# HKUDS/LLMRec

Hardware: NVIDIA H100
Metric: train_interactions_per_sec (higher is better)
Workload: dtype f32

## Files before the change

### llmrec_b200/csrc/proj_tc.cu

```cuda
#include <mutex>
#include <stdlib.h>
#include <vector>
#include <string.h>
#include "common.cuh"
#include "tc_common.cuh"
#include "proj_tc.cuh"

namespace llmrec {

using namespace tc;


typedef CUresult (*EncodeFn)(CUtensorMap*, CUtensorMapDataType, cuuint32_t, void*, const cuuint64_t*, const cuuint64_t*,
                             const cuuint32_t*, const cuuint32_t*, CUtensorMapInterleave, CUtensorMapSwizzle,
                             CUtensorMapL2promotion, CUtensorMapFloatOOBfill);

static EncodeFn get_encode() {
  static EncodeFn fn = nullptr;
  static bool tried = false;
  if (!tried) {
    tried = true;
    void* p = nullptr;
    cudaDriverEntryPointQueryResult q;
    if (cudaGetDriverEntryPoint("cuTensorMapEncodeTiled", &p, cudaEnableDefault, &q) == cudaSuccess && q == cudaDriverEntryPointSuccess)
// ... 54 lines not shown
  a[1] = lds_u32(row + 1024 + c0);
  a[2] = lds_u32(row + c1);
  a[3] = lds_u32(row + 1024 + c1);
}
__device__ __forceinline__ int wgrad_feature(int blk, int warp, int h, int g) {
  return blk * 64 + 32 * (warp >> 1) + 8 * (warp & 1) + 4 * h + (g & 3) + 16 * (g >> 2);
}
__device__ __forceinline__ void ld_frag_wgrad(uint32_t (&a)[4], uint32_t sx, int blk, int kk, int warp, int lane) {
  const int g = lane >> 2, t = lane & 3;
  const uint32_t base = sx + (blk * 2 + (warp >> 1)) * 4096 + kk * 1024 + t * 128 + (g & 3) * 4;
  const uint32_t q = (2 * (warp & 1) + 4 * (g >> 2)) ^ t;
  a[0] = lds_u32(base + (q << 4));
  a[1] = lds_u32(base + ((q ^ 1) << 4));
  a[2] = lds_u32(base + 512 + ((q ^ 4) << 4));
  a[3] = lds_u32(base + 512 + ((q ^ 5) << 4));
}

__device__ __forceinline__ uint32_t i8_pair_bf16(uint32_t w, int b, float s) {
  const float x0 = (__uint_as_float(__byte_perm(w, 0x4B000000u, 0x7650u + b)) - 8388736.0f) * s;
  const float x1 = (__uint_as_float(__byte_perm(w, 0x4B000000u, 0x7651u + b)) - 8388736.0f) * s;
  return __byte_perm(__float_as_uint(x0), __float_as_uint(x1), 0x7632u);
}
__device__ __forceinline__ void i8x16_bf16(const uint4& q, float s, uint4& lo, uint4& hi) {
  const uint32_t w0 = q.x ^ 0x80808080u, w1 = q.y ^ 0x80808080u, w2 = q.z ^ 0x80808080u, w3 = q.w ^ 0x80808080u;
  lo = make_uint4(i8_pair_bf16(w0, 0, s), i8_pair_bf16(w0, 2, s), i8_pair_bf16(w1, 0, s), i8_pair_bf16(w1, 2, s));
  hi = make_uint4(i8_pair_bf16(w2, 0, s), i8_pair_bf16(w2, 2, s), i8_pair_bf16(w3, 0, s), i8_pair_bf16(w3, 2, s));
}
__device__ __forceinline__ void converters_sync() { asm volatile("bar.sync 1, 96;" ::: "memory"); }

template <class Unit>
struct I8Stage {
  static constexpr int kGroups = Unit::Cfg::TM / 64, kTasks = 256;
  static constexpr int kPer = (kTasks + 95) / 96;
  float sc[kPer];
  const float* tile_sc = nullptr;
  __device__ void load_scales(const Unit& w, int kb, int ct) {
#pragma unroll
    for (int m = 0; m < kPer; ++m) {
      const int t = ct + 96 * m;
      sc[m] = t < kTasks ? w.row_scale(w.task_row(0, t, kb)) : 0.f;
    }
  }
  __device__ void expand(uint8_t* sx, int ct) const {
#pragma unroll
    for (int g = 0; g < kGroups; ++g) {
      uint4 v[kPer];
#pragma unroll
      for (int m = 0; m < kPer; ++m) {
        const int t = ct + 96 * m;
        if (t < kTasks) v[m] = *reinterpret_cast<const uint4*>(sx + Unit::Cfg::TM * 64u + g * 4096u + Unit::raw_off(t));
      }
      if (2 * g >= kGroups) converters_sync();
#pragma unroll
      for (int m = 0; m < kPer; ++m) {
        const int t = ct + 96 * m;
        if (t >= kTasks) continue;
        uint4 lo, hi;
        uint32_t o_lo, o_hi;
        i8x16_bf16(v[m], Unit::kScalesPerUnit ? tile_sc[64 * g + (t >> 2)] : sc[m], lo, hi);
        Unit::out_off(t, o_lo, o_hi);
        *reinterpret_cast<uint4*>(sx + g * 8192u + o_lo) = lo;
        *reinterpret_cast<uint4*>(sx + g * 8192u + o_hi) = hi;
      }
    }
  }
};

__device__ __forceinline__ uint32_t i8_raw_off(int t) { return (t >> 2) * 64u + (t & 3) * 16u; }
__device__ __forceinline__ void i8_out_off(int t, uint32_t& lo, uint32_t& hi) {
  const int i = t >> 2, c = 2 * (t & 3);
  lo = i * 128u + (((c ^ i) & 7) << 4);
  hi = i * 128u + ((((c + 1) ^ i) & 7) << 4);
}

__device__ __forceinline__ float i8_row_scale(const RowScales& xs, int p, int n, int row) {
  return row < n ? __ldg(reinterpret_cast<const float*>(xs.scale[p] + (long long)row * xs.pitch[p])) : 0.f;
}

template <int D, bool SPLIT, int MB, bool BF16 = false, bool I8 = false>
struct FwdUnit {
  using Cfg = ProjCfg<D, SPLIT, MB, BF16>;
  static_assert(!I8 || BF16, "int8 X runs the bf16 pipeline");
  static constexpr int kTransA = 0;
  static constexpr int kBuilders = I8 ? 3 : 0;
  static constexpr int kProducerRegs = I8 ? 72 : 40, kConsumerRegs = I8 ? 216 : 232;
  static constexpr uint32_t kRawTx = I8 ? Cfg::TM * 64u : 0u;
  static constexpr uint32_t kTx = I8 ? Cfg::kStage - Cfg::kX : Cfg::kStage;
  const FwdParams& P; int p, mblk, kb_n;
  __device__ FwdUnit(const FwdParams& P_, int u) : P(P_) {
    p = 0;
    while (p + 1 < P.n_prob && u >= P.prob[p + 1].tile_start) ++p;
    mblk = u - P.prob[p].tile_start;
    kb_n = P.prob[p].kblocks;
  }
  __device__ void issue(uint8_t* st, uint64_t* bar, uint64_t* raw_bar, int kb, uint64_t pol) const {
    constexpr int bk = stage_k(BF16);
    if constexpr (I8) tma_load_2d_hint(st + Cfg::TM * 64, &P.tmA[p], raw_bar, kb * bk, mblk * Cfg::TM, pol);
    else tma_load_2d_hint(st, &P.tmA[p], bar, kb * bk, mblk * Cfg::TM, pol);
#pragma unroll
    for (int i = 0; i < Cfg::NB; ++i) tma_load_2d(st + Cfg::kX + i * Cfg::kB, &P.tmW[p], bar, kb * bk, i * D);
  }
  static constexpr bool kScalesPerUnit = true;
  __device__ void tile_scales(float* ts, int ct) const {
    for (int i = ct; i < Cfg::TM; i += 96) ts[i] = i8_row_scale(P.xs, p, P.prob[p].n, mblk * Cfg::TM + i);
  }
  static __device__ uint32_t raw_off(int t) { return i8_raw_off(t); }
  static __device__ void out_off(int t, uint32_t& lo, uint32_t& hi) { i8_out_off(t, lo, hi); }
  static __device__ void ld_frag(uint32_t (&a)[4], uint32_t sx, int blk, int kk, int warp, int lane) { ld_frag_fwd(a, sx, blk, kk, warp, lane); }
  static __device__ uint64_t a_desc(uint32_t sx, int blk, int kk) { return gmma_desc_sw128(sx + blk * 8192u + kk * 32u); }
  __device__ void store(float (&acc)[MB][D / 2], int cw, int warp, int lane) const {
    const FwdProblem& pr = P.prob[p];
    const int g = lane >> 2, t = lane & 3;
#pragma unroll
    for (int j = 0; j < MB; ++j) {
      const int row0 = mblk * Cfg::TM + (cw * MB + j) * 64 + warp * 16 + g;
      long long yrow[2];
#pragma unroll
      for (int h = 0; h < 2; ++h) {
        const int row = row0 + 8 * h;
        yrow[h] = row < pr.n ? (pr.rows ? (long long)__ldg(pr.rows + row) : (long long)row) : -1;
      }
#pragma unroll
      for (int c = 0; c < D / 8; ++c) {
        const int col = c * 8 + 2 * t;
        const float2 b = pr.bias ? __ldg(reinterpret_cast<const float2*>(pr.bias + col)) : make_float2(0.f, 0.f);
#pragma unroll
        for (int h = 0; h < 2; ++h) {
          if (yrow[h] >= 0)
            *reinterpret_cast<float2*>(pr.Y + yrow[h] * pr.ldy + col) = make_float2(acc[j][4 * c + 2 * h] + b.x, acc[j][4 * c + 2 * h + 1] + b.y);
        }
      }
    }
  }
};

template <int D, bool SPLIT, int MB, bool BF16 = false, bool I8 = false>
struct WgUnit {
  using Cfg = ProjCfg<D, SPLIT, MB, BF16>;
  static_assert(!I8 || BF16, "int8 X runs the bf16 pipeline");
  static constexpr int kBk = stage_k(BF16);
  static constexpr int kTransA = 1;
  const WgParams& P; int p, u, ft, r0, kb_n;
  __device__ WgUnit(const WgParams& P_, int u_) : P(P_), u(u_) {
    p = 0;
    while (p + 1 < P.n_prob && u >= P.prob[p + 1].item_start) ++p;
    const WgProblem& pr = P.prob[p];
    const int local = u - pr.item_start, chunk = local / pr.ft_tiles;
    ft = local - chunk * pr.ft_tiles;
    r0 = chunk * pr.rows_per_chunk;
    kb_n = (min(pr.n, r0 + pr.rows_per_chunk) - r0 + kBk - 1) / kBk;
  }
  static constexpr bool kBuildsB = SPLIT && !BF16;
  static constexpr int kBuilders = kBuildsB || I8 ? 3 : 0;
  static constexpr int kProducerRegs = kBuilders ? 72 : 40;
  static constexpr int kConsumerRegs = kBuilders ? 216 : 232;
  static constexpr uint32_t kRawTx = I8 ? Cfg::TM * 64u : 0u;
  static constexpr uint32_t kTx = kBuildsB ? Cfg::kX : I8 ? Cfg::kStage - Cfg::kX : Cfg::kStage;
  __device__ void issue(uint8_t* st, uint64_t* bar, uint64_t* raw_bar, int kb, uint64_t pol) const {
    const int r = r0 + kb * kBk;
    if constexpr (I8) {
#pragma unroll
      for (int b = 0; b < Cfg::TM / 64; ++b) tma_load_2d_hint(st + Cfg::TM * 64 + b * 4096, &P.tmX[p], raw_bar, ft * Cfg::TM + 64 * b, r, pol);
    } else if constexpr (BF16) {
#pragma unroll
      for (int b = 0; b < Cfg::TM / 64; ++b) tma_load_2d_hint(st + b * 8192, &P.tmX[p], bar, ft * Cfg::TM + 64 * b, r, pol);
    } else {
#pragma unroll
      for (int b = 0; b < Cfg::TM / 32; ++b) tma_load_2d_hint(st + b * 4096, &P.tmX[p], bar, ft * Cfg::TM + 32 * b, r, pol);
    }
    if constexpr (!kBuildsB) {
#pragma unroll
      for (int i = 0; i < Cfg::NB; ++i) tma_load_2d(st + Cfg::kX + i * Cfg::kB, &P.tmG[p], bar, r, i * D);
    }
  }
  static constexpr bool kScalesPerUnit = false;
  __device__ void tile_scales(float*, int) const {}
  __device__ int task_row(int, int t, int kb) const { return r0 + kb * kBk + (t >> 2); }
  __device__ float row_scale(int row) const { return i8_row_scale(P.xs, p, P.prob[p].n, row); }
  static __device__ uint32_t raw_off(int t) { return i8_raw_off(t); }
  static __device__ void out_off(int t, uint32_t& lo, uint32_t& hi) { i8_out_off(t, lo, hi); }
  static constexpr int kTasks = D / 8;
  static constexpr int kBatch = 3;
  __device__ void build(uint8_t* st, int kb, int bw, int lane) const {
    const int n = P.prob[p].n, r = r0 + kb * kBk + lane;
    const int* __restrict__ map = P.rows[p];
    const float* src = r < n ? P.dY[p] + (long long)(map ? __ldg(map + r) : r) * P.lddy[p] : nullptr;
    uint8_t* b = st + Cfg::kX + (lane & 3) * 4;
    const int q = lane >> 2;
    for (int t0 = bw; t0 < kTasks; t0 += kBuilders * kBatch) {
      float4 v[kBatch][2];
#pragma unroll
      for (int j = 0; j < kBatch; ++j) {
        const int t = t0 + kBuilders * j;
#pragma unroll
        for (int h = 0; h < 2; ++h)
          v[j][h] = t < kTasks && src ? __ldg(reinterpret_cast<const float4*>(src + 8 * t + 4 * h)) : make_float4(0.f, 0.f, 0.f, 0.f);
      }
#pragma unroll
      for (int j = 0; j < kBatch; ++j) {
        const int t = t0 + kBuilders * j;
        if (t >= kTasks) break;
#pragma unroll
        for (int e = 0; e < 8; ++e) {
          const float4 w = v[j][e >> 2];
          const float x = (e & 3) == 0 ? w.x : (e & 3) == 1 ? w.y : (e & 3) == 2 ? w.z : w.w, hi = tf32_hi(x);
          uint8_t* o = b + (8 * t + e) * 128 + ((q ^ e) & 7) * 16;
          *reinterpret_cast<float*>(o) = hi;
          *reinterpret_cast<float*>(o + Cfg::kB) = x - hi;
        }
      }
    }
  }
  static __device__ void ld_frag(uint32_t (&a)[4], uint32_t sx, int blk, int kk, int warp, int lane) { ld_frag_wgrad(a, sx, blk, kk, warp, lane); }
  static __device__ uint64_t a_desc(uint32_t sx, int blk, int kk) { return gmma_desc_sw128_mn(sx + blk * 8192u + kk * 2048u); }
  __device__ void store(float (&acc)[MB][D / 2], int cw, int warp, int lane) const {
    const int g = lane >> 2, t = lane & 3;
    float* out = P.partial + (long long)u * Cfg::TM * D;
#pragma unroll
    for (int j = 0; j < MB; ++j)
#pragma unroll
      for (int h = 0; h < 2; ++h) {
        const int f = BF16 ? (cw * MB + j) * 64 + warp * 16 + 8 * h + g : wgrad_feature(cw * MB + j, warp, h, g);
        float* o = out + (long long)f * D + 2 * t;
#pragma unroll
        for (int c = 0; c < D / 8; ++c) *reinterpret_cast<float2*>(o + c * 8) = make_float2(acc[j][4 * c + 2 * h], acc[j][4 * c + 2 * h + 1]);
      }
  }
};

template <int D, bool SPLIT, int MB, bool BF16, class Unit, class Params>
__device__ __forceinline__ void proj_pipeline(const Params& P, int total) {
  using Cfg = ProjCfg<D, SPLIT, MB, BF16>;
  extern __shared__ uint8_t smem_raw[];
  uint8_t* smem = align1024(smem_raw);
  uint64_t* full = reinterpret_cast<uint64_t*>(smem + Cfg::kStages * Cfg::kStage);
  uint64_t* empty = full + Cfg::kStages;
  uint64_t* raw = empty + Cfg::kStages;
  float* tile_sc = reinterpret_cast<float*>(raw + Cfg::kStages);
  const int tid = threadIdx.x, wg = tid >> 7, warp = (tid >> 5) & 3, lane = tid & 31;
  if (tid == 0) {
    for (int s = 0; s < Cfg::kStages; ++s) { mbar_init(&full[s], 1 + Unit::kBuilders); mbar_init(&empty[s], 8); mbar_init(&raw[s], 1); }
    fence_barrier_init();
  }
  __syncthreads();

  static_assert(128 * Unit::kProducerRegs + 256 * Unit::kConsumerRegs <= 384 * 168, "setmaxnreg split exceeds the CTA's registers");
  if (wg == 0) {
    setmaxnreg_dec<Unit::kProducerRegs>();
    if (tid == 0) {
      const uint64_t pol = l2_policy_evict_first();
      int s = 0; uint32_t ph = 0;
      for (int u = blockIdx.x; u < total; u += gridDim.x) {
        const Unit w(P, u);
        for (int kb = 0; kb < w.kb_n; ++kb) {
          mbar_wait(&empty[s], ph ^ 1u);
          mbar_arrive_expect_tx(&full[s], Unit::kTx);
          if constexpr (Unit::kRawTx > 0) mbar_arrive_expect_tx(&raw[s], Unit::kRawTx);
          w.issue(smem + s * Cfg::kStage, &full[s], &raw[s], kb, pol);
          if (++s == Cfg::kStages) { s = 0; ph ^= 1u; }
        }
      }
    }
    if constexpr (Unit::kBuilders > 0) {
      if (warp >= 1) {
        int s = 0; uint32_t ph = 0;
        for (int u = blockIdx.x; u < total; u += gridDim.x) {
          const Unit w(P, u);
          [[maybe_unused]] I8Stage<Unit> cv;
          if constexpr (Unit::kRawTx > 0 && Unit::kScalesPerUnit) {
            converters_sync();
            w.tile_scales(tile_sc, tid - 32);
            converters_sync();
            cv.tile_sc = tile_sc;
          }
          for (int kb = 0; kb < w.kb_n; ++kb) {
            if constexpr (Unit::kRawTx > 0) {
              if constexpr (!Unit::kScalesPerUnit) cv.load_scales(w, kb, tid - 32);
              mbar_wait(&raw[s], ph);
              cv.expand(smem + s * Cfg::kStage, tid - 32);
            } else {
              mbar_wait(&empty[s], ph ^ 1u);
              w.build(smem + s * Cfg::kStage, kb, warp - 1, lane);
            }
            fence_proxy_async_smem();
            __syncwarp();
            if (lane == 0) mbar_arrive(&full[s]);
            if (++s == Cfg::kStages) { s = 0; ph ^= 1u; }
          }
        }
      }
    }
    return;
  }

  setmaxnreg_inc<Unit::kConsumerRegs>();
  const int cw = wg - 1;
  int s = 0; uint32_t ph = 0;
  float acc[MB][D / 2];
  for (int u = blockIdx.x; u < total; u += gridDim.x) {
    const Unit w(P, u);
#pragma unroll
    for (int j = 0; j < MB; ++j)
#pragma unroll
      for (int i = 0; i < D / 2; ++i) acc[j][i] = 0.f;
    int prev = -1;
    for (int kb = 0; kb < w.kb_n; ++kb) {
      mbar_wait(&full[s], ph);
      const uint32_t st = smem_u32(smem + s * Cfg::kStage), bh = st + Cfg::kX, bl = bh + Cfg::kB;
      if constexpr (BF16) {
#pragma unroll
        for (int kk = 0; kk < 4; ++kk) {
          wgmma_fence();
#pragma unroll
          for (int j = 0; j < MB; ++j) {
            const uint64_t a = Unit::a_desc(st, cw * MB + j, kk);
            if (SPLIT) {
              WgmmaSSbf16<D, Unit::kTransA>::mma(acc[j], a, gmma_desc_sw128(bl + Cfg::kB + kk * 32u));
              WgmmaSSbf16<D, Unit::kTransA>::mma(acc[j], a, gmma_desc_sw128(bl + kk * 32u));
            }
            WgmmaSSbf16<D, Unit::kTransA>::mma(acc[j], a, gmma_desc_sw128(bh + kk * 32u));
          }
          wgmma_commit();
          wgmma_wait<1>();
          if (kk == 0 && prev >= 0 && lane == 0) mbar_arrive(&empty[prev]);
        }
      } else {
#pragma unroll
        for (int kk = 0; kk < 4; ++kk) {
          uint32_t ah[MB][4], al[MB][4];
#pragma unroll
          for (int j = 0; j < MB; ++j) {
            Unit::ld_frag(ah[j], st, cw * MB + j, kk, warp, lane);
            if (SPLIT)
#pragma unroll
              for (int i = 0; i < 4; ++i) {
                const float x = __uint_as_float(ah[j][i]), hi = tf32_hi(x);
                ah[j][i] = __float_as_uint(hi);
                al[j][i] = __float_as_uint(x - hi);
              }
          }
          wgmma_fence();
          const uint64_t dh = gmma_desc_sw128(bh + kk * 32u);
#pragma unroll
          for (int j = 0; j < MB; ++j) {
            if (SPLIT) {
              WgmmaRS<D>::mma(acc[j], al[j], dh);
              WgmmaRS<D>::mma(acc[j], ah[j], gmma_desc_sw128(bl + kk * 32u));
            }
            WgmmaRS<D>::mma(acc[j], ah[j], dh);
          }
          wgmma_commit();
          wgmma_wait<1>();
          if (kk == 0 && prev >= 0 && lane == 0) mbar_arrive(&empty[prev]);
        }
      }
      prev = s;
      if (++s == Cfg::kStages) { s = 0; ph ^= 1u; }
    }
    wgmma_wait<0>();
    if (prev >= 0 && lane == 0) mbar_arrive(&empty[prev]);
    w.store(acc, cw, warp, lane);
  }
}

template <int D, bool SPLIT, int MB, XType XT>
__global__ void __launch_bounds__(384, 1) proj_fwd_tc_kernel(const __grid_constant__ FwdParams P) {
  constexpr bool BF16 = XT != XType::F32;
  proj_pipeline<D, SPLIT, MB, BF16, FwdUnit<D, SPLIT, MB, BF16, XT == XType::I8>>(P, P.total_tiles);
}

template <int D, bool SPLIT, int MB, XType XT>
__global__ void __launch_bounds__(384, 1) proj_wgrad_tc_kernel(const __grid_constant__ WgParams P) {
  constexpr bool BF16 = XT != XType::F32;
  proj_pipeline<D, SPLIT, MB, BF16, WgUnit<D, SPLIT, MB, BF16, XT == XType::I8>>(P, P.total_items);
}

static int num_sms() {
  static int n[64] = {};
  int dev = 0;
  if (cudaGetDevice(&dev) != cudaSuccess || dev < 0 || dev >= 64) return 132;
  if (!n[dev] && cudaDeviceGetAttribute(&n[dev], cudaDevAttrMultiProcessorCount, dev) != cudaSuccess) n[dev] = 132;
  return n[dev];
// ... 137 lines not shown
#pragma unroll 4
    for (int c = 0; c < pr.chunks; ++c, ++idx) {
      if ((idx & 3) != sl) continue;
      const float4 v = __ldg(reinterpret_cast<const float4*>(R.partial + ((long long)(pr.item_start + c * pr.ft_tiles + ft) * tm + f) * d) + dc4);
      s.x += v.x; s.y += v.y; s.z += v.z; s.w += v.w;
    }
  }
  part[sl][e] = s;
  __syncthreads();
  if (sl == 0 && owned) {
    float4 a = part[0][e], b = part[1][e], c = part[2][e], g = part[3][e];
    float4 t = make_float4((a.x + b.x) + (c.x + g.x), (a.y + b.y) + (c.y + g.y), (a.z + b.z) + (c.z + g.z), (a.w + b.w) + (c.w + g.w));
    const int gf = ft * tm + f;
    if (gf < ro.k) {
      float* p = ro.dW + (long long)(dc4 * 4) * ro.k + gf;
      if (ro.accumulate) { t.x += p[0]; t.y += p[ro.k]; t.z += p[2LL * ro.k]; t.w += p[3LL * ro.k]; }
      p[0] = t.x; p[ro.k] = t.y; p[2LL * ro.k] = t.z; p[3LL * ro.k] = t.w;
    }
  }
}

struct ColsumParams { const float* dY[kMaxProb]; long long ld[kMaxProb]; long long n[kMaxProb]; float* db[kMaxProb]; int acc[kMaxProb]; int d; int n_prob; float* partial; unsigned* ticket; };
constexpr int kColsumSlices = 128;
__global__ void __launch_bounds__(256) colsum_kernel(const ColsumParams P) {
  __shared__ float red[256];
  __shared__ bool s_last;
  const int p = blockIdx.y, b = blockIdx.x, d = P.d;
  const int groups = 256 / d > 0 ? 256 / d : 1;
  const int g = threadIdx.x / d, c = threadIdx.x - g * d;
  float s = 0.f;
  if (g < groups && P.db[p]) {
#pragma unroll 4
    for (long long r = (long long)b * groups + g; r < P.n[p]; r += (long long)kColsumSlices * groups) s += __ldg(P.dY[p] + r * P.ld[p] + c);
  }
  red[threadIdx.x] = (g < groups) ? s : 0.f;
  __syncthreads();
  if (threadIdx.x < d) {
    float t = 0.f;
    for (int gg = 0; gg < groups; ++gg) t += red[gg * d + threadIdx.x];
    P.partial[((long long)p * kColsumSlices + b) * d + threadIdx.x] = t;
  }
  __threadfence();
  __syncthreads();
  if (threadIdx.x == 0) s_last = atomicAdd(P.ticket, 1u) == gridDim.x * gridDim.y - 1;
  __syncthreads();
  if (!s_last) return;
  __threadfence();
  for (int q = 0; q < P.n_prob; ++q) {
    if (!P.db[q]) continue;
    float t = 0.f;
    if (g < groups)
      for (int bb = g; bb < kColsumSlices; bb += groups) t += __ldcg(P.partial + ((long long)q * kColsumSlices + bb) * d + c);
    __syncthreads();
    red[threadIdx.x] = (g < groups) ? t : 0.f;
    __syncthreads();
    if (threadIdx.x < d) {
      float u = 0.f;
      for (int gg = 0; gg < groups; ++gg) u += red[gg * d + threadIdx.x];
      float* o = P.db[q] + threadIdx.x;
      *o = P.acc[q] ? (*o + u) : u;
    }
  }
  if (threadIdx.x == 0) *P.ticket = 0u;
}

bool proj_tc_supported(int d, int64_t ldx, const void* X, int k, bool wgrad, XType xt) {
  (void)wgrad;
  const int q = xt == XType::I8 ? 16 : xt == XType::BF16 ? 8 : 4;
  return d % 32 == 0 && d >= 32 && d <= 256 && ldx % q == 0 && aligned16(X) && k >= 1 && k % q == 0;
}

static CUtensorMapDataType x_type(bool bf16) { return bf16 ? CU_TENSOR_MAP_DATA_TYPE_BFLOAT16 : CU_TENSOR_MAP_DATA_TYPE_FLOAT32; }

static bool x_tmap(CUtensorMap* m, XType xt, const void* X, int k, int64_t n, int64_t ldx, uint32_t box_k, uint32_t box_rows) {
  if (xt == XType::I8) return make_tmap_2d(m, CU_TENSOR_MAP_DATA_TYPE_UINT8, X, (uint64_t)k, (uint64_t)n, (uint64_t)ldx, box_k, box_rows, false);
  return make_tmap_2d(m, x_type(xt == XType::BF16), X, (uint64_t)k, (uint64_t)n, (uint64_t)ldx * (xt == XType::BF16 ? 2 : 4), box_k, box_rows);
}

static void set_row_scales(RowScales& xs, int p, XType xt, const void* X, int k, int64_t ldx) {
  xs.scale[p] = xt == XType::I8 ? static_cast<const uint8_t*>(X) + i8_scale_offset(k) : nullptr;
  xs.pitch[p] = xt == XType::I8 ? ldx : 0;
}

int proj_fwd_tc_group(const llmrec_proj_fwd_problem* pr, const int32_t* const* rows, int n_prob, int d, int mode, XType xt, cudaStream_t st) {
  const bool split = (mode == 0), bf16 = xt != XType::F32;
  const bool need_ws = split || bf16;
  const int es = bf16 ? 2 : 4, bk = stage_k(bf16);
  FwdParams P;
  memset(&P, 0, sizeof(P));
  P.n_prob = n_prob; P.d = d;
  WsplitParams WS;
  memset(&WS, 0, sizeof(WS));
  int n_ws = 0;
  long long ws_max = 0, tiles256 = 0;
  for (int p = 0; p < n_prob; ++p) tiles256 += (pr[p].n + tile_m(2) - 1) / tile_m(2);
  const int mb = pick_mb(d, tiles256), tm = tile_m(mb);
  int tiles = 0;
  for (int p = 0; p < n_prob; ++p) {
    const float* wsrc = need_ws ? pr[p].wsplit : pr[p].W;
    LLMREC_CHECK_ARG(!need_ws || pr[p].wsplit, "proj_fwd: 3xTF32 mode and bf16 X need a wsplit buffer of 2*d*k floats");
    bool fresh = true;
    for (int q = 0; q < p; ++q) fresh = fresh && !(pr[q].W == pr[p].W && pr[q].wsplit == pr[p].wsplit);
    if (need_ws && fresh) {
      WS.W[n_ws] = pr[p].W; WS.out[n_ws] = pr[p].wsplit; WS.n[n_ws] = (long long)d * pr[p].k;
      ws_max = WS.n[n_ws] > ws_max ? WS.n[n_ws] : ws_max;
      ++n_ws;
    }
    if (pr[p].n > 0) {
      const int pieces = split ? (bf16 ? 3 : 2) : 1;
      if (!x_tmap(&P.tmA[p], xt, pr[p].X, pr[p].k, pr[p].n, pr[p].ldx, bk, (uint32_t)tm)) return 4;
      if (!make_tmap_2d(&P.tmW[p], x_type(bf16), wsrc, (uint64_t)pr[p].k, (uint64_t)(pieces * d), (uint64_t)pr[p].k * es, bk, (uint32_t)d)) return 4;
    }
    P.prob[p].n = (int)pr[p].n; P.prob[p].k = pr[p].k; P.prob[p].kblocks = (pr[p].k + bk - 1) / bk;
    P.prob[p].tile_start = tiles; P.prob[p].ldy = pr[p].ldy; P.prob[p].Y = pr[p].Y; P.prob[p].bias = pr[p].bias;
    P.prob[p].rows = rows ? rows[p] : nullptr;
    set_row_scales(P.xs, p, xt, pr[p].X, pr[p].k, pr[p].ldx);
    tiles += (int)((pr[p].n + tm - 1) / tm);
  }
  P.total_tiles = tiles;
  if (n_ws > 0) {
    if (bf16) wsplit_bf16_kernel<<<dim3((unsigned)((ws_max + 255) / 256), n_ws), 256, 0, st>>>(WS, split ? 1 : 0);
    else wsplit_kernel<<<dim3((unsigned)((ws_max + 255) / 256), n_ws), 256, 0, st>>>(WS);
    LLMREC_CHECK_LAUNCH("wsplit");
  }
  if (tiles <= 0) return 0;
  return fwd_launch(P, split, mb, xt, st);
}

static int wg_rows_per_chunk(int64_t n) {
  int r = 2048;
  while (r > 256 && n / r < 4) r >>= 1;
  return r;
}

struct WgPlan { WgProblem prob[kMaxProb]; int items, mb, tm; int64_t ldt[kMaxProb], dyt[kMaxProb], colsum, total; };
static bool wg_builds_b(int mode, bool bf16) { return mode == 0 && !bf16; }
static void wg_plan(const llmrec_proj_wgrad_problem* pr, int n_prob, int d, int mode, bool bf16, WgPlan& W) {
  long long items256 = 0;
  for (int p = 0; p < n_prob; ++p) {
    const int rpc = wg_rows_per_chunk(pr[p].n);
    items256 += (long long)((pr[p].k + tile_m(2) - 1) / tile_m(2)) * ((pr[p].n + rpc - 1) / rpc);
  }
  W.mb = pick_mb(d, items256); W.tm = tile_m(W.mb);
  W.items = 0;
  for (int p = 0; p < n_prob; ++p) {
    WgProblem& w = W.prob[p];
    w.n = (int)pr[p].n; w.k = pr[p].k; w.ft_tiles = (pr[p].k + W.tm - 1) / W.tm;
    w.rows_per_chunk = wg_rows_per_chunk(pr[p].n);
    w.chunks = (int)((pr[p].n + w.rows_per_chunk - 1) / w.rows_per_chunk);
    w.item_start = W.items;
    W.items += w.ft_tiles * w.chunks;
  }
  W.colsum = 4 + (int64_t)W.items * W.tm * d;
  int64_t off = W.colsum + (int64_t)n_prob * kColsumSlices * d;
  for (int p = 0; p < n_prob; ++p) {
    W.ldt[p] = bf16 ? (pr[p].n + 7) & ~int64_t(7) : (pr[p].n + 3) & ~int64_t(3);
    W.dyt[p] = off;
    if (!wg_builds_b(mode, bf16)) off += 2 * (int64_t)d * W.ldt[p];
  }
  W.total = off;
}

int64_t proj_wgrad_tc_scratch(const llmrec_proj_wgrad_problem* pr, int n_prob, int d, int mode, XType xt) {
  WgPlan W;
  wg_plan(pr, n_prob, d, mode, xt != XType::F32, W);
  return W.total;
}

int proj_wgrad_tc_group(const llmrec_proj_wgrad_problem* pr, const int32_t* const* rows, const int64_t* n_dy, int n_prob, int d, int mode,
                        XType xt, float* scratch, int64_t scratch_elems, cudaStream_t st) {
  const bool split = (mode == 0), bf16 = xt != XType::F32;
  const int es = bf16 ? 2 : 4, bk = stage_k(bf16), pieces = split ? (bf16 ? 3 : 2) : 1;
  const bool build_b = wg_builds_b(mode, bf16);
  WgPlan W;
  wg_plan(pr, n_prob, d, mode, bf16, W);
  LLMREC_CHECK_ARG(scratch && scratch_elems >= W.total, "proj_wgrad: scratch too small (%lld < %lld)", (long long)scratch_elems, (long long)W.total);
  WgParams P;
  memset(&P, 0, sizeof(P));
  P.n_prob = n_prob; P.d = d; P.total_items = W.items;
  P.partial = scratch + 4;
  ColsumParams C;
  memset(&C, 0, sizeof(C));
  C.d = d; C.n_prob = n_prob; C.partial = scratch + W.colsum;
  C.ticket = reinterpret_cast<unsigned*>(scratch);
  DytParams T;
  memset(&T, 0, sizeof(T));
  T.d = d; T.split = split ? 1 : 0;
  int64_t n_max = 0;
  for (int p = 0; p < n_prob; ++p) {
    P.prob[p] = W.prob[p];
    const int32_t* map = rows ? rows[p] : nullptr;
    float* dyt = scratch + W.dyt[p];
    if (pr[p].n > 0) {
      if (!x_tmap(&P.tmX[p], xt, pr[p].X, pr[p].k, pr[p].n, pr[p].ldx, bk, bk)) return 4;
      if (!build_b &&
          !make_tmap_2d(&P.tmG[p], x_type(bf16), dyt, (uint64_t)pr[p].n, (uint64_t)(pieces * d), (uint64_t)W.ldt[p] * es, bk, (uint32_t)d)) return 4;
    }
    P.dY[p] = pr[p].dY; P.lddy[p] = pr[p].lddy; P.rows[p] = map;
    set_row_scales(P.xs, p, xt, pr[p].X, pr[p].k, pr[p].ldx);
    T.dY[p] = pr[p].dY; T.ld[p] = pr[p].lddy; T.n[p] = (int)pr[p].n; T.out[p] = dyt; T.ldt[p] = W.ldt[p]; T.rows[p] = map;
    n_max = pr[p].n > n_max ? pr[p].n : n_max;
    C.dY[p] = pr[p].dY; C.ld[p] = pr[p].lddy; C.n[p] = n_dy ? n_dy[p] : pr[p].n; C.db[p] = pr[p].db;
    C.acc[p] = pr[p].accumulate & LLMREC_WGRAD_ACCUMULATE;
  }
  bool any_db = false;
  for (int p = 0; p < n_prob; ++p) any_db = any_db || pr[p].db != nullptr;
  static const bool branches = !(getenv("LLMREC_BRANCHES") && atoi(getenv("LLMREC_BRANCHES")) == 0);
  struct Branch { cudaStream_t side; cudaEvent_t fork, join; };
  static Branch per_device[64] = {};
  int dev = 0;
  LLMREC_CHECK_CUDA(cudaGetDevice(&dev));
  LLMREC_CHECK_ARG(dev >= 0 && dev < 64, "proj_wgrad: device ordinal %d out of range", dev);
  cudaStream_t& side = per_device[dev].side;
  cudaEvent_t& ev_fork = per_device[dev].fork;
  cudaEvent_t& ev_join = per_device[dev].join;
  bool forked = false;
  if (any_db) {
    cudaStream_t cs = st;
    if (branches) {
      if (!side) {
        LLMREC_CHECK_CUDA(cudaStreamCreateWithFlags(&side, cudaStreamNonBlocking));
        LLMREC_CHECK_CUDA(cudaEventCreateWithFlags(&ev_fork, cudaEventDisableTiming));
        LLMREC_CHECK_CUDA(cudaEventCreateWithFlags(&ev_join, cudaEventDisableTiming));
      }
      LLMREC_CHECK_CUDA(cudaEventRecord(ev_fork, st));
      LLMREC_CHECK_CUDA(cudaStreamWaitEvent(side, ev_fork, 0));
      cs = side; forked = true;
    }
    colsum_kernel<<<dim3(kColsumSlices, n_prob), 256, 0, cs>>>(C);
    LLMREC_CHECK_LAUNCH("colsum");
    if (forked) LLMREC_CHECK_CUDA(cudaEventRecord(ev_join, side));
  }
  if (W.items > 0) {
    if (!build_b) {
      const dim3 grid((unsigned)((n_max + 31) / 32), (unsigned)(d / 32), (unsigned)n_prob);
      if (bf16) dyt_split_kernel<true><<<grid, 256, 0, st>>>(T);
      else dyt_split_kernel<false><<<grid, 256, 0, st>>>(T);
      LLMREC_CHECK_LAUNCH("dyt_split");
    }
    int rc = wgrad_launch(P, split, W.mb, xt, st);
    if (rc) return rc;
  }
  ReduceParams R;
  memset(&R, 0, sizeof(R));
  R.d = d; R.tm = W.tm; R.partial = scratch + 4;
  int blocks = 0;
  for (int p = 0; p < n_prob; ++p) {
    R.prob[p] = P.prob[p];
    int o = -1;
    for (int q = 0; q < R.n_out; ++q) if (R.out[q].dW == pr[p].dW) o = q;
    if (o < 0) {
      o = R.n_out++;
      R.out[o].dW = pr[p].dW; R.out[o].k = pr[p].k; R.out[o].accumulate = pr[p].accumulate & LLMREC_WGRAD_ACCUMULATE; R.out[o].n_src = 0;
    }
    LLMREC_CHECK_ARG(R.out[o].k == pr[p].k, "proj_wgrad: problems sharing dW must share k");
    R.out[o].src[R.out[o].n_src++] = p;
  }
  const int feats_per_blk = 64 / (d / 4);
  for (int o = 0; o < R.n_out; ++o) { R.out[o].blk_start = blocks; blocks += ((R.out[o].k + W.tm - 1) / W.tm) * (W.tm / feats_per_blk); }
  wgrad_reduce_kernel<<<blocks, 256, 0, st>>>(R);
  LLMREC_CHECK_LAUNCH("wgrad_reduce");
  if (forked) LLMREC_CHECK_CUDA(cudaStreamWaitEvent(st, ev_join, 0));
  return 0;
}

}
```

### llmrec_b200/ops.py

```python
from __future__ import annotations

import copy
import ctypes as C
import os

import numpy as np
import torch

from . import _native as N
from . import feat_int8


STATS = {"launches": 0}


def _count(n=1):
    STATS["launches"] += n


def _stream():
    return C.c_void_p(torch.cuda.current_stream().cuda_stream)


def _p(t):
# ... 195 lines not shown
        return k
    return int(X.shape[1])


_PROBLEMS = {torch.float32: (N.ProjFwdProblem, N.ProjWgradProblem, "f32"), torch.bfloat16: (N.ProjFwdProblemBf16, N.ProjWgradProblemBf16, "bf16"),
             torch.int8: (N.ProjFwdProblemI8, N.ProjWgradProblemI8, "i8")}


def _group_dtype(Xs, what):
    dt = {X.dtype for X in Xs}
    if len(dt) != 1:
        raise ValueError(f"{what}: every problem of one call must share the X dtype, got {sorted(str(t) for t in dt)}")
    return dt.pop()


def _f32(t, name):
    if t is not None and t.dtype != torch.float32:
        raise ValueError(f"{name}: must be fp32 (only the feature table X may be bf16 or int8), got {t.dtype}")
    return t


def _row_map(rows, n, what):
    if rows is not None and (_i32(rows, what + " rows").dim() != 1 or rows.numel() != n):
        raise ValueError(f"{what}: a row map needs one entry per X row ({n}), got {tuple(rows.shape)}")
    return rows


def _problem_array(prob_type, n, mapped):
    if not mapped:
        arr = (prob_type * n)()
        return arr, None, arr

    class Block(C.Structure):
        _fields_ = [("probs", prob_type * n), ("maps", N.ProjRowMap * n)]
    blk = Block()
    return blk.probs, blk.maps, blk


def proj_fwd_group(problems, d, mode=0):
    dt = _group_dtype([_feat(pr[0]) for pr in problems], "proj_fwd")
    bf16 = dt != torch.float32
    prob_t, _, suffix = _PROBLEMS[dt]
    arr, recs, _blk = _problem_array(prob_t, len(problems), any(len(pr) > 4 and pr[4] is not None for pr in problems))
    for i, (X, W, b, out, *rows) in enumerate(problems):
        _mat(out); _f32(W, "proj_fwd W"); _f32(b, "proj_fwd bias")
        n, k = int(X.shape[0]), _feat_k(X, int(W.shape[1]) if W.dim() == 2 else -1, "proj_fwd")
        rows = _row_map(rows[0] if rows else None, n, "proj_fwd")
        if not W.is_contiguous() or tuple(W.shape) != (d, k) or out.shape[1] != d or (rows is None and out.shape[0] != n):
            raise ValueError("proj_fwd: bad shapes")
        ws = _get_scratch(("wsplit", W.data_ptr()), 2 * d * k, X.device) if mode == 0 or (bf16 and mode == 1) else None
        arr[i] = prob_t(_p(X), _p(W), _p(b), _p(out), _p(ws), _ld(X), _ld(out), n, k, 0 if rows is None else N.PROJ_ROW_MAP)
        if rows is not None:
            recs[i] = N.ProjRowMap(_p(rows), int(out.shape[0]))
    lib = N.lib()
    if bf16:
        N.check(getattr(lib, "llmrec_proj_fwd_group_" + suffix)(arr, len(problems), d, mode, _stream()), "proj_fwd_group_" + suffix)
    else:
        N.check(lib.llmrec_proj_fwd_group_f32(arr, len(problems), d, mode, _stream()), "proj_fwd_group")
    _count((2 if mode == 0 or (bf16 and mode == 1) else 1) * -(-len(problems) // 8))


def proj_fwd(X, W, b, out, mode=0):
    proj_fwd_group([(X, W, b, out)], W.shape[0], mode)
    return out


def proj_wgrad_group(problems, d, mode=0):
    dt = _group_dtype([_feat(pr[0]) for pr in problems], "proj_wgrad")
    _, prob_t, suffix = _PROBLEMS[dt]
    arr, recs, _blk = _problem_array(prob_t, len(problems), any(len(pr) > 5 and pr[5] is not None for pr in problems))
    for i, (X, dY, dW, db, acc, *rows) in enumerate(problems):
        _mat(dY); _f32(dW, "proj_wgrad dW"); _f32(db, "proj_wgrad db")
        n, k = int(X.shape[0]), _feat_k(X, int(dW.shape[1]) if dW.dim() == 2 else -1, "proj_wgrad")
        rows = _row_map(rows[0] if rows else None, n, "proj_wgrad")
        if not dW.is_contiguous() or tuple(dW.shape) != (d, k) or dY.shape[1] != d or (rows is None and dY.shape[0] != n):
            raise ValueError("proj_wgrad: bad shapes")
        flags = (N.WGRAD_ACCUMULATE if acc else 0) | (0 if rows is None else N.PROJ_ROW_MAP)
        arr[i] = prob_t(_p(X), _p(dY), _p(dW), _p(db), _ld(X), _ld(dY), n, k, flags)
        if rows is not None:
            recs[i] = N.ProjRowMap(_p(rows), int(dY.shape[0]))
    lib = N.lib()
    name = "llmrec_proj_wgrad_group" + ("" if dt == torch.float32 else "_" + suffix)
    need = int(getattr(lib, name + "_scratch")(arr, len(problems), d, mode))
    scratch = _get_scratch(("wgrad", problems[0][0].device.index), need, problems[0][0].device, zero=True) if need else None
    if dt != torch.float32:
        N.check(getattr(lib, name)(arr, len(problems), d, mode, _p(scratch), need, _stream()), "proj_wgrad_group_" + suffix)
    else:
        N.check(lib.llmrec_proj_wgrad_group_f32(arr, len(problems), d, mode, _p(scratch), need, _stream()), "proj_wgrad_group")
    _count(4 if need else len(problems))


def proj_wgrad(X, dY, dW, db, accumulate=False, mode=0):
    proj_wgrad_group([(X, dY, dW, db, accumulate)], dY.shape[1], mode)


def _ptr_table(tensors):
    arr = (C.c_void_p * max(1, len(tensors)))()
    for i, t in enumerate(tensors):
        arr[i] = t.data_ptr() if t is not None else None
    return arr


def _ld_table(tensors):
    arr = (C.c_int64 * max(1, len(tensors)))()
    for i, t in enumerate(tensors):
        arr[i] = _ld(t) if t is not None else 0
    return arr


def _row_list(rows, count, max_rows, what):
    if rows is None:
        raise ValueError(f"{what}: a device-side count needs a row list")
    mx = int(rows.numel()) if max_rows is None else min(int(max_rows), int(rows.numel()))
    return _i32(rows), _i32(count, "count"), mx


def fuse_fwd(layers, sides, coefs, out, rows=None, compact=False, count=None, max_rows=None):
    for t in list(layers) + list(sides) + [out]:
        _mat(t)
    cf = (C.c_float * max(1, len(coefs)))(*[float(c) for c in coefs])
    if count is not None:
        if compact:
            raise ValueError("fuse_fwd: the device-count form is not compact")
        rows, count, mx = _row_list(rows, count, max_rows, "fuse_fwd")
        N.check(N.lib().llmrec_fuse_fwd_rows_f32(_ptr_table(layers), _ld_table(layers), len(layers), _ptr_table(sides), _ld_table(sides), cf,
                                                  len(sides), _p(out), _ld(out), _p(rows), _p(count), mx, out.shape[1], _stream()), "fuse_fwd_rows")
        _count()
        return out
    n = out.shape[0] if rows is None else rows.numel()
    if compact:
        if rows is None:
            raise ValueError("fuse_fwd: compact form needs a row list")
        n = -n
    N.check(N.lib().llmrec_fuse_fwd_f32(_ptr_table(layers), _ld_table(layers), len(layers), _ptr_table(sides), _ld_table(sides), cf,
                                         len(sides), _p(out), _ld(out), _p(rows), n, out.shape[1], _stream()), "fuse_fwd")
    _count()
    return out


def fuse_bwd(g, n_layers, d_layer, sides, coefs, d_sides, accumulate, rows=None, count=None, max_rows=None):
    _mat(g)
    cf = (C.c_float * max(1, len(coefs)))(*[float(c) for c in coefs])
    dl = (_p(d_layer), _ld(d_layer) if d_layer is not None else 0)
    if count is not None:
        rows, count, mx = _row_list(rows, count, max_rows, "fuse_bwd")
        N.check(N.lib().llmrec_fuse_bwd_rows_f32(_p(g), _ld(g), n_layers, *dl, _ptr_table(sides), _ld_table(sides), cf, _ptr_table(d_sides),
                                                  _ld_table(d_sides), len(sides), 1 if accumulate else 0, _p(rows), _p(count), mx, g.shape[1],
                                                  _stream()), "fuse_bwd_rows")
        _count()
        return
    n = g.shape[0] if rows is None else rows.numel()
    N.check(N.lib().llmrec_fuse_bwd_f32(_p(g), _ld(g), n_layers, *dl,
                                         _ptr_table(sides), _ld_table(sides), cf, _ptr_table(d_sides), _ld_table(d_sides), len(sides),
                                         1 if accumulate else 0, _p(rows), n, g.shape[1], _stream()), "fuse_bwd")
    _count()


def bpr_work(n_heads, B, device):
    return torch.zeros(int(N.lib().llmrec_bpr_work_elems(n_heads, B)), dtype=torch.float32, device=device)


def bpr_slot_plan(users, pos, neg, meta=None, plan=None):
    B = int(users.numel())
    need = int(N.lib().llmrec_bpr_slot_plan_elems(B))
    if plan is None:
        plan = torch.zeros(need, dtype=torch.int32, device=users.device)
    if _i32(plan, "plan").numel() < need:
# ... 228 lines not shown
```

Baseline: 1.336 million.

## Run wgrad GEMM on high-priority side stream with per-stream branch slots

Side streams and events become per caller stream (up to eight slots per device, guarded by a mutex), and a high-priority stream is added. The wgrad GEMM now runs on that stream, forked from and joined back to the caller stream, so it can be scheduled ahead of concurrent work. The scratch buffer is keyed by the dW pointer rather than the device, so concurrent wgrad groups no longer share scratch. This adds event and stream overhead per call and allocates more scratch memory.

```diff
diff --git a/llmrec_b200/csrc/proj_tc.cu b/llmrec_b200/csrc/proj_tc.cu
--- a/llmrec_b200/csrc/proj_tc.cu
+++ b/llmrec_b200/csrc/proj_tc.cu
@@ -803,30 +803,47 @@
   bool any_db = false;
   for (int p = 0; p < n_prob; ++p) any_db = any_db || pr[p].db != nullptr;
   static const bool branches = !(getenv("LLMREC_BRANCHES") && atoi(getenv("LLMREC_BRANCHES")) == 0);
-  struct Branch { cudaStream_t side; cudaEvent_t fork, join; };
-  static Branch per_device[64] = {};
+  constexpr int kSlots = 8;
+  struct Branch { bool used; cudaStream_t owner, side, hi; cudaEvent_t fork, join, hfork, hjoin; };
+  static Branch per_device[64][kSlots] = {};
+  static std::mutex slots_mu;
   int dev = 0;
   LLMREC_CHECK_CUDA(cudaGetDevice(&dev));
   LLMREC_CHECK_ARG(dev >= 0 && dev < 64, "proj_wgrad: device ordinal %d out of range", dev);
-  cudaStream_t& side = per_device[dev].side;
-  cudaEvent_t& ev_fork = per_device[dev].fork;
-  cudaEvent_t& ev_join = per_device[dev].join;
+  Branch* br = nullptr;
+  if (any_db && branches) {
+    std::lock_guard<std::mutex> lock(slots_mu);
+    Branch* slots = per_device[dev];
+    if (!slots[0].side)
+      for (int i = 0; i < kSlots; ++i) {
+        LLMREC_CHECK_CUDA(cudaStreamCreateWithFlags(&slots[i].side, cudaStreamNonBlocking));
+        LLMREC_CHECK_CUDA(cudaEventCreateWithFlags(&slots[i].fork, cudaEventDisableTiming));
+        LLMREC_CHECK_CUDA(cudaEventCreateWithFlags(&slots[i].join, cudaEventDisableTiming));
+        int lo = 0, hi = 0;
+        LLMREC_CHECK_CUDA(cudaDeviceGetStreamPriorityRange(&lo, &hi));
+        LLMREC_CHECK_CUDA(cudaStreamCreateWithPriority(&slots[i].hi, cudaStreamNonBlocking, hi));
+        LLMREC_CHECK_CUDA(cudaEventCreateWithFlags(&slots[i].hfork, cudaEventDisableTiming));
+        LLMREC_CHECK_CUDA(cudaEventCreateWithFlags(&slots[i].hjoin, cudaEventDisableTiming));
+      }
+    for (int i = 0; i < kSlots && !br; ++i) {
+      if (slots[i].used && slots[i].owner == st) br = &slots[i];
+      else if (!slots[i].used) { slots[i].used = true; slots[i].owner = st; br = &slots[i]; }
+    }
+  }
   bool forked = false;
+  cudaEvent_t ev_join = nullptr;
   if (any_db) {
     cudaStream_t cs = st;
-    if (branches) {
-      if (!side) {
-        LLMREC_CHECK_CUDA(cudaStreamCreateWithFlags(&side, cudaStreamNonBlocking));
-        LLMREC_CHECK_CUDA(cudaEventCreateWithFlags(&ev_fork, cudaEventDisableTiming));
-        LLMREC_CHECK_CUDA(cudaEventCreateWithFlags(&ev_join, cudaEventDisableTiming));
-      }
-      LLMREC_CHECK_CUDA(cudaEventRecord(ev_fork, st));
-      LLMREC_CHECK_CUDA(cudaStreamWaitEvent(side, ev_fork, 0));
+    if (br) {
+      cudaStream_t side = br->side;
+      ev_join = br->join;
+      LLMREC_CHECK_CUDA(cudaEventRecord(br->fork, st));
+      LLMREC_CHECK_CUDA(cudaStreamWaitEvent(side, br->fork, 0));
       cs = side; forked = true;
     }
     colsum_kernel<<<dim3(kColsumSlices, n_prob), 256, 0, cs>>>(C);
     LLMREC_CHECK_LAUNCH("colsum");
-    if (forked) LLMREC_CHECK_CUDA(cudaEventRecord(ev_join, side));
+    if (forked) LLMREC_CHECK_CUDA(cudaEventRecord(ev_join, cs));
   }
   if (W.items > 0) {
     if (!build_b) {
@@ -835,7 +852,11 @@
       else dyt_split_kernel<false><<<grid, 256, 0, st>>>(T);
       LLMREC_CHECK_LAUNCH("dyt_split");
     }
-    int rc = wgrad_launch(P, split, W.mb, xt, st);
+    const bool hp = br != nullptr;
+    cudaStream_t ws = hp ? br->hi : st;
+    if (hp) { LLMREC_CHECK_CUDA(cudaEventRecord(br->hfork, st)); LLMREC_CHECK_CUDA(cudaStreamWaitEvent(ws, br->hfork, 0)); }
+    int rc = wgrad_launch(P, split, W.mb, xt, ws);
+    if (hp) { LLMREC_CHECK_CUDA(cudaEventRecord(br->hjoin, ws)); LLMREC_CHECK_CUDA(cudaStreamWaitEvent(st, br->hjoin, 0)); }
     if (rc) return rc;
   }
   ReduceParams R;
diff --git a/llmrec_b200/ops.py b/llmrec_b200/ops.py
--- a/llmrec_b200/ops.py
+++ b/llmrec_b200/ops.py
@@ -301,7 +301,7 @@
     lib = N.lib()
     name = "llmrec_proj_wgrad_group" + ("" if dt == torch.float32 else "_" + suffix)
     need = int(getattr(lib, name + "_scratch")(arr, len(problems), d, mode))
-    scratch = _get_scratch(("wgrad", problems[0][0].device.index), need, problems[0][0].device, zero=True) if need else None
+    scratch = _get_scratch(("wgrad", problems[0][2].data_ptr()), need, problems[0][0].device, zero=True) if need else None
     if dt != torch.float32:
         N.check(getattr(lib, name)(arr, len(problems), d, mode, _p(scratch), need, _stream()), "proj_wgrad_group_" + suffix)
     else:
```

Measured after the change: 1.339 million (median of 6 runs). Within noise of the previous version (+0.2%).

## Snake-order forward projection tiles and pick tile height from simulated per-CTA load

Applied to the files above, without the earlier changes.

Forward projection units are now assigned to CTAs in boustrophedon (snake) order: odd rounds reverse the block-to-tile mapping, which evens out the work each persistent CTA receives. For f32 inputs where the default heuristic picks MB=2, a host-side simulation of per-CTA load under snake scheduling compares 128-row and 256-row tiles, and switches to MB=1 if that lowers the maximum load by more than about 4%. The goal is to reduce tail imbalance across SMs. The cost is some extra host work per call, and smaller tiles if the switch is taken.

```diff
diff --git a/llmrec_b200/csrc/proj_tc.cu b/llmrec_b200/csrc/proj_tc.cu
--- a/llmrec_b200/csrc/proj_tc.cu
+++ b/llmrec_b200/csrc/proj_tc.cu
@@ -160,6 +160,7 @@
   using Cfg = ProjCfg<D, SPLIT, MB, BF16>;
   static_assert(!I8 || BF16, "int8 X runs the bf16 pipeline");
   static constexpr int kTransA = 0;
+  static constexpr bool kSnake = true;
   static constexpr int kBuilders = I8 ? 3 : 0;
   static constexpr int kProducerRegs = I8 ? 72 : 40, kConsumerRegs = I8 ? 216 : 232;
   static constexpr uint32_t kRawTx = I8 ? Cfg::TM * 64u : 0u;
@@ -218,6 +219,7 @@
   static_assert(!I8 || BF16, "int8 X runs the bf16 pipeline");
   static constexpr int kBk = stage_k(BF16);
   static constexpr int kTransA = 1;
+  static constexpr bool kSnake = false;
   const WgParams& P; int p, u, ft, r0, kb_n;
   __device__ WgUnit(const WgParams& P_, int u_) : P(P_), u(u_) {
     p = 0;
@@ -306,6 +308,12 @@
   }
 };
 
+template <bool SNAKE>
+__device__ __forceinline__ int cta_unit(int r) {
+  const int G = gridDim.x, b = blockIdx.x;
+  return r * G + (SNAKE && (r & 1) ? G - 1 - b : b);
+}
+
 template <int D, bool SPLIT, int MB, bool BF16, class Unit, class Params>
 __device__ __forceinline__ void proj_pipeline(const Params& P, int total) {
   using Cfg = ProjCfg<D, SPLIT, MB, BF16>;
@@ -328,7 +336,7 @@
     if (tid == 0) {
       const uint64_t pol = l2_policy_evict_first();
       int s = 0; uint32_t ph = 0;
-      for (int u = blockIdx.x; u < total; u += gridDim.x) {
+      for (int r = 0, u; (u = cta_unit<Unit::kSnake>(r)) < total; ++r) {
         const Unit w(P, u);
         for (int kb = 0; kb < w.kb_n; ++kb) {
           mbar_wait(&empty[s], ph ^ 1u);
@@ -342,7 +350,7 @@
     if constexpr (Unit::kBuilders > 0) {
       if (warp >= 1) {
         int s = 0; uint32_t ph = 0;
-        for (int u = blockIdx.x; u < total; u += gridDim.x) {
+        for (int r = 0, u; (u = cta_unit<Unit::kSnake>(r)) < total; ++r) {
           const Unit w(P, u);
           [[maybe_unused]] I8Stage<Unit> cv;
           if constexpr (Unit::kRawTx > 0 && Unit::kScalesPerUnit) {
@@ -375,7 +383,7 @@
   const int cw = wg - 1;
   int s = 0; uint32_t ph = 0;
   float acc[MB][D / 2];
-  for (int u = blockIdx.x; u < total; u += gridDim.x) {
+  for (int r = 0, u; (u = cta_unit<Unit::kSnake>(r)) < total; ++r) {
     const Unit w(P, u);
 #pragma unroll
     for (int j = 0; j < MB; ++j)
@@ -679,6 +687,31 @@
   xs.pitch[p] = xt == XType::I8 ? ldx : 0;
 }
 
+static long long fwd_max_load(const llmrec_proj_fwd_problem* pr, int n_prob, int tm, int bk) {
+  long long units = 0;
+  for (int p = 0; p < n_prob; ++p) units += (pr[p].n + tm - 1) / tm;
+  const int G = (int)(units < num_sms() ? units : num_sms());
+  std::vector<long long> load(G > 0 ? G : 1, 0);
+  long long u = 0;
+  for (int p = 0; p < n_prob; ++p) {
+    const long long cost = (long long)((pr[p].k + bk - 1) / bk) * (tm / 128);
+    for (long long t = 0; t < (pr[p].n + tm - 1) / tm; ++t, ++u) {
+      const long long r = u / G, b = u % G;
+      load[(r & 1) ? G - 1 - b : b] += cost;
+    }
+  }
+  long long mx = 0;
+  for (long long l : load) mx = l > mx ? l : mx;
+  return mx;
+}
+
+static int fwd_pick_mb(const llmrec_proj_fwd_problem* pr, int n_prob, int d, XType xt, long long tiles256) {
+  const int mb = pick_mb(d, tiles256);
+  if (mb != 2 || xt != XType::F32) return mb;
+  const int bk = stage_k(false);
+  return 25 * fwd_max_load(pr, n_prob, tile_m(1), bk) < 24 * fwd_max_load(pr, n_prob, tile_m(2), bk) ? 1 : 2;
+}
+
 int proj_fwd_tc_group(const llmrec_proj_fwd_problem* pr, const int32_t* const* rows, int n_prob, int d, int mode, XType xt, cudaStream_t st) {
   const bool split = (mode == 0), bf16 = xt != XType::F32;
   const bool need_ws = split || bf16;
@@ -691,7 +724,7 @@
   int n_ws = 0;
   long long ws_max = 0, tiles256 = 0;
   for (int p = 0; p < n_prob; ++p) tiles256 += (pr[p].n + tile_m(2) - 1) / tile_m(2);
-  const int mb = pick_mb(d, tiles256), tm = tile_m(mb);
+  const int mb = fwd_pick_mb(pr, n_prob, d, xt, tiles256), tm = tile_m(mb);
   int tiles = 0;
   for (int p = 0; p < n_prob; ++p) {
     const float* wsrc = need_ws ? pr[p].wsplit : pr[p].W;
```

Result: faster. 1.360 million before, 1.381 million after (median of 6 runs) (+1.6%).
